# ChenRocks/UNITER

Measured on NVIDIA H100. Metric: uniter_base_encoder_fwd_bwd_samples_per_sec, higher is better.
Workload: dtype bf16

## Files before the change

uniter_b200/csrc/attn.cu:

```cuda
#include "common.h"
#include "ptx.cuh"
#include "wgmma.cuh"

namespace ub {

constexpr int ATT_D = 64;
constexpr int ATT_BM = 128;
constexpr int ATT_BN = 128;
constexpr int ATT_TILE = ATT_BM * ATT_D * 2;
constexpr int ATT_MAXSEQ = 512;
constexpr int ATT_THREADS = 256;

struct AttnParams {
  const int* cu_seqlens;
  int B, H, nheads, T;
  void* ctx;
  float* lse;
  float scale;
  uint32_t drop_thr16;
  float drop_inv_keep;
  uint32_t seed_lo, seed_hi, stream_lo, stream_hi;
  const void* dctx;
  void* dqkv;
  float* dbias;
  const unsigned long long* rng_dev;
};


__device__ __forceinline__ void frag_colsum64_atomic(const float (&d)[32], bool ok0, bool ok1, float* dst,
                                                     int lane) {
#pragma unroll
  for (int jj = 0; jj < 8; ++jj) {
#pragma unroll
    for (int t = 0; t < 2; ++t) {
      float x = (ok0 ? d[4 * jj + t] : 0.f) + (ok1 ? d[4 * jj + 2 + t] : 0.f);
      x += __shfl_xor_sync(0xffffffffu, x, 4);
      x += __shfl_xor_sync(0xffffffffu, x, 8);
      x += __shfl_xor_sync(0xffffffffu, x, 16);
      if (lane < 4) atomicAdd(dst + 8 * jj + 2 * lane + t, x);
    }
  }
}

__device__ __forceinline__ void frag_colsum64_warp(const float (&d)[32], bool ok0, bool ok1, float* dst, int lane) {
#pragma unroll
  for (int jj = 0; jj < 8; ++jj) {
#pragma unroll
    for (int t = 0; t < 2; ++t) {
      float x = (ok0 ? d[4 * jj + t] : 0.f) + (ok1 ? d[4 * jj + 2 + t] : 0.f);
      x += __shfl_xor_sync(0xffffffffu, x, 4);
      x += __shfl_xor_sync(0xffffffffu, x, 8);
      x += __shfl_xor_sync(0xffffffffu, x, 16);
      if (lane < 4) dst[8 * jj + 2 * lane + t] += x;
    }
  }
}

template <bool kBF16>
__device__ __forceinline__ void store_frag_row(void* out_row, const float (&d)[32], int e, int q4, float mul) {
  uint32_t* o = reinterpret_cast<uint32_t*>(out_row);
#pragma unroll
  for (int jj = 0; jj < 8; ++jj)
    o[(8 * jj + 2 * q4) >> 1] = Elem<kBF16>::pack(d[4 * jj + 2 * e] * mul, d[4 * jj + 2 * e + 1] * mul);
}

__device__ __forceinline__ uint64_t attn_drop_group(int bh, int q, int key8) {
  return ((static_cast<uint64_t>(bh) * ATT_MAXSEQ + q) * ATT_MAXSEQ + key8) >> 3;
}

__device__ __forceinline__ void quad_drop_words(const DropoutRng& rng, int bh, int q, int key_base, int jb,
                                                int lane, uint32_t (&w)[4]) {
  const int q4 = lane & 3;
  const uint4 r = rng.draw8(attn_drop_group(bh, q, key_base + 8 * (4 * jb + q4)));
  uint32_t got[4];
#pragma unroll
  for (int k = 0; k < 4; ++k) {
    const int sw = (q4 - k) & 3;
    const uint32_t v = sw == 0 ? r.x : (sw == 1 ? r.y : (sw == 2 ? r.z : r.w));
    got[k] = __shfl_sync(0xffffffffu, v, (lane & ~3) | ((q4 + k) & 3));
  }
#pragma unroll
  for (int t = 0; t < 4; ++t) {
    const int k = (t - q4) & 3;
    w[t] = k == 0 ? got[0] : (k == 1 ? got[1] : (k == 2 ? got[2] : got[3]));
  }
}

__device__ __forceinline__ uint32_t rand16_half(uint32_t w, int t) { return t ? (w >> 16) : (w & 0xFFFFu); }

__device__ __forceinline__ void st_swz128_u32(uint8_t* base, int r, int col, uint32_t v) {
  const int slab = col >> 6;
  const int chunk = (col & 63) >> 3;
  uint8_t* p = base + slab * ATT_TILE + r * 128 + ((chunk ^ (r & 7)) << 4) + (col & 7) * 2;
  *reinterpret_cast<uint32_t*>(p) = v;
}

template <bool kBF16>
__device__ __forceinline__ void row_delta_lse(const AttnParams& p, int seq0, int head, int row, bool ok, int q4,
                                              float& delta, float& lse2) {
  using T16 = typename Elem<kBF16>::T;
  float d = 0.f;
  lse2 = 0.f;
  if (ok) {
    const size_t off = static_cast<size_t>(seq0 + row) * p.H + head * ATT_D + 16 * q4;
    const uint4* g_do = reinterpret_cast<const uint4*>(reinterpret_cast<const T16*>(p.dctx) + off);
    const uint4* g_o = reinterpret_cast<const uint4*>(reinterpret_cast<const T16*>(p.ctx) + off);
#pragma unroll
    for (int v = 0; v < 2; ++v) {
      const uint4 a = __ldg(g_do + v), o = __ldg(g_o + v);
      float2 x, y;
      x = Elem<kBF16>::unpack(a.x); y = Elem<kBF16>::unpack(o.x); d += x.x * y.x + x.y * y.y;
      x = Elem<kBF16>::unpack(a.y); y = Elem<kBF16>::unpack(o.y); d += x.x * y.x + x.y * y.y;
      x = Elem<kBF16>::unpack(a.z); y = Elem<kBF16>::unpack(o.z); d += x.x * y.x + x.y * y.y;
      x = Elem<kBF16>::unpack(a.w); y = Elem<kBF16>::unpack(o.w); d += x.x * y.x + x.y * y.y;
    }
    lse2 = p.lse[static_cast<size_t>(head) * p.T + seq0 + row] * 1.4426950408889634f;
  }
  d += __shfl_xor_sync(0xffffffffu, d, 1);
  d += __shfl_xor_sync(0xffffffffu, d, 2);
  delta = d;
}

constexpr int SH_TILE = 64 * ATT_D * 2;
constexpr int SH_THREADS = 128;
constexpr int SH_MAXSEQ = 128;

__device__ __forceinline__ void wg_sync() { asm volatile("bar.sync 1, 128;" ::: "memory"); }

__device__ __forceinline__ int seq_blocks(const int* cu, int b) { return min((cu[b + 1] - cu[b] + 63) >> 6, 2); }

struct ShortSched {
  const int* cu;
  int B, nheads, h, b;
  long long start, hi;

  __device__ bool valid() const { return h < nheads && start < hi; }
  __device__ int blocks() const { return seq_blocks(cu, b); }

  __device__ void init(const int* cu_, int B_, int nheads_, int lane) {
    cu = cu_; B = B_; nheads = nheads_;
    h = nheads; start = hi = 0;
    int wb = 0;
    for (int b0 = 0; b0 < B; b0 += 32) {
      int c = b0 + lane < B ? seq_blocks(cu, b0 + lane) : 0;
      c *= c;
#pragma unroll
      for (int d = 16; d >= 1; d >>= 1) c += __shfl_xor_sync(0xffffffffu, c, d);
      wb += c;
    }
    if (wb == 0) return;
    const long long W = static_cast<long long>(nheads) * wb;
    const long long lo = W * blockIdx.x / gridDim.x;
    hi = W * (blockIdx.x + 1) / gridDim.x;
    if (lo >= hi) return;
    const int hh = static_cast<int>(lo / wb);
    const long long r = lo - static_cast<long long>(hh) * wb;
    int pref = 0;
    for (int b0 = 0; b0 < B; b0 += 32) {
      int c = b0 + lane < B ? seq_blocks(cu, b0 + lane) : 0;
      c *= c;
      int incl = c;
#pragma unroll
      for (int d = 1; d < 32; d <<= 1) {
        const int t = __shfl_up_sync(0xffffffffu, incl, d);
        if (lane >= d) incl += t;
      }
      const int excl = pref + incl - c;
      const unsigned m = __ballot_sync(0xffffffffu, b0 + lane < B && excl >= r);
      if (m) {
        const int L = __ffs(m) - 1;
        h = hh;
        b = b0 + L;
        start = static_cast<long long>(hh) * wb + __shfl_sync(0xffffffffu, excl, L);
        skip_empty();
        return;
      }
      pref += __shfl_sync(0xffffffffu, incl, 31);
    }
    h = hh + 1;
    b = 0;
    start = static_cast<long long>(h) * wb;
    skip_empty();
  }
  __device__ void step() {
    const int nb = blocks();
    start += nb * nb;
    if (++b == B) { b = 0; ++h; }
  }
  __device__ void skip_empty() {
    while (valid() && cu[b + 1] == cu[b]) step();
  }
  __device__ void next() { step(); skip_empty(); }
};

template <bool kBF16, int NB>
__device__ __forceinline__ void attn_fwd_short_rows(const AttnParams& p, uint32_t uQ, uint32_t uK, uint32_t uV,
                                                    int qb, int S, int seq0, int head, int bh,
                                                    const DropoutRng& rng, int warp, int lane) {
  const int q4 = lane & 3;
  const float c = p.scale * 1.4426950408889634f;
  int qrow[2];
#pragma unroll
  for (int e = 0; e < 2; ++e) qrow[e] = 64 * qb + 16 * warp + (lane >> 2) + 8 * e;

  float s[NB][32];
  wgmma_fence();
#pragma unroll
  for (int kb = 0; kb < NB; ++kb)
#pragma unroll
    for (int k = 0; k < ATT_D / 16; ++k)
      Wgmma<64, kBF16, 0, 0>::ss(s[kb], gmma_desc(uQ + qb * SH_TILE + k * 32, 16, 1024),
                                 gmma_desc(uK + kb * SH_TILE + k * 32, 16, 1024), k != 0);
  wgmma_commit();
  wgmma_wait<0>();

  float m[2] = {-INFINITY, -INFINITY}, l[2] = {0.f, 0.f};
#pragma unroll
  for (int kb = 0; kb < NB; ++kb)
#pragma unroll
    for (int i = 0; i < 32; ++i) {
      const int key = 64 * kb + 8 * (i >> 2) + 2 * q4 + (i & 1);
      if (key < S) m[(i >> 1) & 1] = fmaxf(m[(i >> 1) & 1], s[kb][i]);
    }
#pragma unroll
  for (int e = 0; e < 2; ++e) {
    m[e] = fmaxf(m[e], __shfl_xor_sync(0xffffffffu, m[e], 1));
    m[e] = fmaxf(m[e], __shfl_xor_sync(0xffffffffu, m[e], 2));
  }
  const float mc[2] = {m[0] * c, m[1] * c};

#pragma unroll
  for (int kb = 0; kb < NB; ++kb) {
#pragma unroll
    for (int jb = 0; jb < 2; ++jb) {
      uint32_t dw[2][4];
#pragma unroll
      for (int e = 0; e < 2; ++e)
        if (p.drop_thr16) quad_drop_words(rng, bh, qrow[e], 64 * kb, jb, lane, dw[e]);
#pragma unroll
      for (int jq = 0; jq < 4; ++jq) {
        const int jj = 4 * jb + jq;
#pragma unroll
        for (int e = 0; e < 2; ++e) {
#pragma unroll
          for (int t = 0; t < 2; ++t) {
            const int i = 4 * jj + 2 * e + t;
            const int key = 64 * kb + 8 * jj + 2 * q4 + t;
            float pv = key < S ? ex2_approx(fmaf(s[kb][i], c, -mc[e])) : 0.f;
            l[e] += pv;
            if (p.drop_thr16) {
              const float pr = Elem<kBF16>::to_f(Elem<kBF16>::from_f(pv));
              pv = (rand16_half(dw[e][jq], t) < p.drop_thr16) ? 0.f : pr * p.drop_inv_keep;
            }
            s[kb][i] = pv;
          }
        }
      }
    }
  }

  float o[32];
  wgmma_fence();
#pragma unroll
  for (int kb = 0; kb < NB; ++kb)
#pragma unroll
    for (int kk = 0; kk < 4; ++kk) {
      const uint32_t a[4] = {Elem<kBF16>::pack(s[kb][8 * kk + 0], s[kb][8 * kk + 1]),
                             Elem<kBF16>::pack(s[kb][8 * kk + 2], s[kb][8 * kk + 3]),
                             Elem<kBF16>::pack(s[kb][8 * kk + 4], s[kb][8 * kk + 5]),
                             Elem<kBF16>::pack(s[kb][8 * kk + 6], s[kb][8 * kk + 7])};
      Wgmma<64, kBF16, 0, 1>::rs(o, a, gmma_desc(uV + kb * SH_TILE + kk * 2048, 8192, 1024), (kb | kk) != 0);
    }
  wgmma_commit();
  wgmma_wait<0>();

#pragma unroll
  for (int e = 0; e < 2; ++e) {
    l[e] += __shfl_xor_sync(0xffffffffu, l[e], 1);
    l[e] += __shfl_xor_sync(0xffffffffu, l[e], 2);
    if (qrow[e] >= S) continue;
    if (q4 == 0) p.lse[static_cast<size_t>(head) * p.T + seq0 + qrow[e]] = m[e] * p.scale + logf(l[e]);
    typename Elem<kBF16>::T* out = reinterpret_cast<typename Elem<kBF16>::T*>(p.ctx) +
                                   static_cast<size_t>(seq0 + qrow[e]) * p.H + head * ATT_D;
    store_frag_row<kBF16>(out, o, e, q4, 1.f / l[e]);
  }
}

template <bool kBF16>
__global__ void __launch_bounds__(SH_THREADS, 2)
attn_fwd_short_kernel(const __grid_constant__ CUtensorMap tmQKV64, const AttnParams p) {
  pdl_launch_dependents();
  pdl_wait();
  extern __shared__ __align__(1024) uint8_t smem_raw[];
  uint8_t* smem = smem_raw + ((1024u - (smem_u32(smem_raw) & 1023u)) & 1023u);
  uint8_t* sQ = smem;
  uint8_t* sK = smem + 2 * SH_TILE;
  uint8_t* sV = smem + 4 * SH_TILE;
  uint64_t* bar = reinterpret_cast<uint64_t*>(smem + 6 * SH_TILE);

  const int tid = threadIdx.x, warp = tid >> 5, lane = tid & 31;
  if (tid == 0) {
    tma_prefetch_desc(&tmQKV64);
    mbar_init(&bar[0], 1);
    mbar_init(&bar[1], 1);
    fence_barrier_init();
  }
  wg_sync();
  uint32_t rs0 = p.stream_lo, rs1 = p.stream_hi;
  if (p.drop_thr16) rng_add_dev_offset(p.rng_dev, rs0, rs1);
  DropoutRng rng;
  rng.k0 = p.seed_lo; rng.k1 = p.seed_hi; rng.s0 = rs0; rng.s1 = rs1;

  auto load = [&](const ShortSched& it, int slot) {
    const int seq0 = p.cu_seqlens[it.b], nb = it.blocks(), col = it.h * ATT_D;
    mbar_expect_tx(&bar[slot], nb * 3 * SH_TILE);
    for (int r = 0; r < nb; ++r) {
      const int o = (slot + r) * SH_TILE;
      tma_load_2d(sQ + o, &tmQKV64, &bar[slot], col, seq0 + 64 * r);
      tma_load_2d(sK + o, &tmQKV64, &bar[slot], p.H + col, seq0 + 64 * r);
      tma_load_2d(sV + o, &tmQKV64, &bar[slot], 2 * p.H + col, seq0 + 64 * r);
    }
  };

  ShortSched it;
  it.init(p.cu_seqlens, p.B, p.nheads, lane);
  if (it.valid() && tid == 0) load(it, 0);
  int slot = 0;
  uint32_t ph = 0;
  while (it.valid()) {
    ShortSched nx = it;
    nx.next();
    const int seq0 = p.cu_seqlens[it.b], S = p.cu_seqlens[it.b + 1] - seq0, nb = it.blocks();
    const bool pre = nx.valid() && nb == 1 && nx.blocks() == 1;
    const int nslot = pre ? slot ^ 1 : 0;
    if (pre && tid == 0) load(nx, nslot);
    mbar_wait(&bar[slot], (ph >> slot) & 1);
    ph ^= 1u << slot;
    const uint32_t uQ = smem_u32(sQ + slot * SH_TILE), uK = smem_u32(sK + slot * SH_TILE),
                   uV = smem_u32(sV + slot * SH_TILE);
    const int bh = it.b * p.nheads + it.h;
    if (nb == 1) {
      attn_fwd_short_rows<kBF16, 1>(p, uQ, uK, uV, 0, S, seq0, it.h, bh, rng, warp, lane);
    } else {
#pragma unroll 1
      for (int qb = 0; qb < 2; ++qb)
        attn_fwd_short_rows<kBF16, 2>(p, uQ, uK, uV, qb, S, seq0, it.h, bh, rng, warp, lane);
    }
    wg_sync();
    if (nx.valid() && !pre && tid == 0) load(nx, 0);
    it = nx;
    slot = nslot;
  }
}

constexpr int SH_FWD_SMEM = 6 * SH_TILE + 16 + 1024;

template <bool kBF16, int NB>
__device__ __forceinline__ void dq_block(float (&dq)[32], uint32_t uDS, uint32_t uK, int qb) {
  wgmma_fence();
#pragma unroll
  for (int kk = 0; kk < 4 * NB; ++kk)
    Wgmma<64, kBF16, 0, 1>::ss(dq, gmma_desc(uDS + (qb * NB + (kk >> 2)) * SH_TILE + (kk & 3) * 32, 16, 1024),
                               gmma_desc(uK + kk * 2048, 8192, 1024), kk != 0);
  wgmma_commit();
  wgmma_wait<0>();
}

template <bool kBF16, bool kBias = true>
__global__ void __launch_bounds__(SH_THREADS, 2)
attn_bwd_short_kernel(const __grid_constant__ CUtensorMap tmQKV64, const __grid_constant__ CUtensorMap tmDO64,
                      const AttnParams p) {
  using T16 = typename Elem<kBF16>::T;
  pdl_launch_dependents();
  pdl_wait();
  extern __shared__ __align__(1024) uint8_t smem_raw[];
  __shared__ float sBias[4][3 * ATT_D];
  uint8_t* smem = smem_raw + ((1024u - (smem_u32(smem_raw) & 1023u)) & 1023u);
  uint8_t* sQ = smem;
  uint8_t* sK = smem + 2 * SH_TILE;
  uint8_t* sV = smem + 4 * SH_TILE;
  uint8_t* sdO = smem + 6 * SH_TILE;
  uint8_t* sP = smem + 8 * SH_TILE;
  uint8_t* sDS = smem + 9 * SH_TILE;
  uint64_t* bar = reinterpret_cast<uint64_t*>(smem + 13 * SH_TILE);

  const int tid = threadIdx.x, warp = tid >> 5, lane = tid & 31, q4 = lane & 3;
  if (tid == 0) {
    tma_prefetch_desc(&tmQKV64);
    tma_prefetch_desc(&tmDO64);
    mbar_init(&bar[0], 1);
    mbar_init(&bar[1], 1);
    fence_barrier_init();
  }
  for (int i = tid; i < 4 * 3 * ATT_D; i += SH_THREADS) (&sBias[0][0])[i] = 0.f;
  wg_sync();
  uint32_t rs0 = p.stream_lo, rs1 = p.stream_hi;
  if (p.drop_thr16) rng_add_dev_offset(p.rng_dev, rs0, rs1);
  DropoutRng rng;
  rng.k0 = p.seed_lo; rng.k1 = p.seed_hi; rng.s0 = rs0; rng.s1 = rs1;
  const float c = p.scale * 1.4426950408889634f;
  int r_loc[2];
#pragma unroll
  for (int e = 0; e < 2; ++e) r_loc[e] = 16 * warp + (lane >> 2) + 8 * e;
  const uint32_t uP = smem_u32(sP), uDS = smem_u32(sDS);

  auto load = [&](const ShortSched& it, int slot) {
    const int seq0 = p.cu_seqlens[it.b], nb = it.blocks(), col = it.h * ATT_D;
    mbar_expect_tx(&bar[slot], nb * 4 * SH_TILE);
    for (int r = 0; r < nb; ++r) {
      const int o = (slot + r) * SH_TILE;
      tma_load_2d(sQ + o, &tmQKV64, &bar[slot], col, seq0 + 64 * r);
      tma_load_2d(sK + o, &tmQKV64, &bar[slot], p.H + col, seq0 + 64 * r);
      tma_load_2d(sV + o, &tmQKV64, &bar[slot], 2 * p.H + col, seq0 + 64 * r);
      tma_load_2d(sdO + o, &tmDO64, &bar[slot], col, seq0 + 64 * r);
    }
  };

  ShortSched it;
  it.init(p.cu_seqlens, p.B, p.nheads, lane);
  if (it.valid() && tid == 0) load(it, 0);
  int slot = 0;
  uint32_t ph = 0;
  while (it.valid()) {
    ShortSched nx = it;
    nx.next();
    const int seq0 = p.cu_seqlens[it.b], S = p.cu_seqlens[it.b + 1] - seq0, nb = it.blocks();
    const int head = it.h, bh = it.b * p.nheads + head;
    const bool pre = nx.valid() && nb == 1 && nx.blocks() == 1;
    const int nslot = pre ? slot ^ 1 : 0;
    if (pre && tid == 0) load(nx, nslot);
    mbar_wait(&bar[slot], (ph >> slot) & 1);
    ph ^= 1u << slot;
    const uint32_t uQ = smem_u32(sQ + slot * SH_TILE), udO = smem_u32(sdO + slot * SH_TILE),
                   uK = smem_u32(sK + slot * SH_TILE), uV = smem_u32(sV + slot * SH_TILE);

    for (int kb = 0; kb < nb; ++kb) {
      float dv[32], dk[32];
      for (int qb = 0; qb < nb; ++qb) {
        int qrow[2];
        bool q_ok[2];
        float delta[2], lse2[2];
#pragma unroll
        for (int e = 0; e < 2; ++e) {
          qrow[e] = 64 * qb + r_loc[e];
          q_ok[e] = qrow[e] < S;
          row_delta_lse<kBF16>(p, seq0, head, qrow[e], q_ok[e], q4, delta[e], lse2[e]);
        }
        float s[32], dp[32];
        wgmma_fence();
#pragma unroll
        for (int k = 0; k < ATT_D / 16; ++k)
          Wgmma<64, kBF16, 0, 0>::ss(s, gmma_desc(uQ + qb * SH_TILE + k * 32, 16, 1024),
                                     gmma_desc(uK + kb * SH_TILE + k * 32, 16, 1024), k != 0);
#pragma unroll
        for (int k = 0; k < ATT_D / 16; ++k)
          Wgmma<64, kBF16, 0, 0>::ss(dp, gmma_desc(udO + qb * SH_TILE + k * 32, 16, 1024),
                                     gmma_desc(uV + kb * SH_TILE + k * 32, 16, 1024), k != 0);
        wgmma_commit();
        wgmma_wait<0>();

        uint8_t* dsTile = sDS + (qb * nb + kb) * SH_TILE;
#pragma unroll
        for (int jb = 0; jb < 2; ++jb) {
          uint32_t dw[2][4];
#pragma unroll
          for (int e = 0; e < 2; ++e)
            if (p.drop_thr16) quad_drop_words(rng, bh, qrow[e], 64 * kb, jb, lane, dw[e]);
#pragma unroll
          for (int jq = 0; jq < 4; ++jq) {
            const int jj = 4 * jb + jq;
#pragma unroll
            for (int e = 0; e < 2; ++e) {
              float pd[2], ds[2];
#pragma unroll
              for (int t = 0; t < 2; ++t) {
                const int idx = 4 * jj + 2 * e + t;
                const bool ok = q_ok[e] && 64 * kb + 8 * jj + 2 * q4 + t < S;
                float pr = ok ? ex2_approx(fmaf(s[idx], c, -lse2[e])) : 0.f;
                pr = Elem<kBF16>::to_f(Elem<kBF16>::from_f(pr));
                float dpv = dp[idx];
                float pdv = pr;
                if (p.drop_thr16) {
                  const bool drop = rand16_half(dw[e][jq], t) < p.drop_thr16;
                  pdv = drop ? 0.f : pr * p.drop_inv_keep;
                  dpv = drop ? 0.f : dpv * p.drop_inv_keep;
                }
                pd[t] = pdv;
                ds[t] = ok ? pr * (dpv - delta[e]) * p.scale : 0.f;
              }
              st_swz128_u32(sP, r_loc[e], 8 * jj + 2 * q4, Elem<kBF16>::pack(pd[0], pd[1]));
              st_swz128_u32(dsTile, r_loc[e], 8 * jj + 2 * q4, Elem<kBF16>::pack(ds[0], ds[1]));
            }
          }
        }
        fence_proxy_async_smem();
        wg_sync();

        const uint32_t uDSt = smem_u32(dsTile);
        wgmma_fence();
#pragma unroll
        for (int kk = 0; kk < 4; ++kk)
          Wgmma<64, kBF16, 1, 1>::ss(dv, gmma_desc(uP + kk * 2048, SH_TILE, 1024),
                                     gmma_desc(udO + qb * SH_TILE + kk * 2048, 8192, 1024), (qb | kk) != 0);
#pragma unroll
        for (int kk = 0; kk < 4; ++kk)
          Wgmma<64, kBF16, 1, 1>::ss(dk, gmma_desc(uDSt + kk * 2048, SH_TILE, 1024),
                                     gmma_desc(uQ + qb * SH_TILE + kk * 2048, 8192, 1024), (qb | kk) != 0);
        wgmma_commit();
        wgmma_wait<0>();
        wg_sync();
      }
      int key[2];
      bool k_ok[2];
#pragma unroll
      for (int e = 0; e < 2; ++e) {
        key[e] = 64 * kb + r_loc[e];
        k_ok[e] = key[e] < S;
      }
      if (kBias && p.dbias) {
        frag_colsum64_warp(dk, k_ok[0], k_ok[1], sBias[warp] + ATT_D, lane);
        frag_colsum64_warp(dv, k_ok[0], k_ok[1], sBias[warp] + 2 * ATT_D, lane);
      }
#pragma unroll
      for (int e = 0; e < 2; ++e) {
        if (!k_ok[e]) continue;
        T16* outk = reinterpret_cast<T16*>(p.dqkv) + static_cast<size_t>(seq0 + key[e]) * (3 * p.H) + p.H +
                    head * ATT_D;
        store_frag_row<kBF16>(outk, dk, e, q4, 1.f);
        store_frag_row<kBF16>(outk + p.H, dv, e, q4, 1.f);
      }
    }

    for (int qb = 0; qb < nb; ++qb) {
      float dq[32];
      if (nb == 1) dq_block<kBF16, 1>(dq, uDS, uK, 0);
      else dq_block<kBF16, 2>(dq, uDS, uK, qb);
      bool q_ok[2];
#pragma unroll
      for (int e = 0; e < 2; ++e) q_ok[e] = 64 * qb + r_loc[e] < S;
      if (kBias && p.dbias) frag_colsum64_warp(dq, q_ok[0], q_ok[1], sBias[warp], lane);
#pragma unroll
      for (int e = 0; e < 2; ++e)
        if (q_ok[e])
          store_frag_row<kBF16>(reinterpret_cast<T16*>(p.dqkv) + static_cast<size_t>(seq0 + 64 * qb + r_loc[e]) *
                                                                       (3 * p.H) + head * ATT_D,
                                dq, e, q4, 1.f);
    }
    wg_sync();
    if (nx.valid() && !pre && tid == 0) load(nx, 0);
    if (kBias && p.dbias && (!nx.valid() || nx.h != head)) {
      for (int i = tid; i < 3 * ATT_D; i += SH_THREADS) {
        atomicAdd(p.dbias + (i >> 6) * p.H + head * ATT_D + (i & 63),
                  (sBias[0][i] + sBias[1][i]) + (sBias[2][i] + sBias[3][i]));
        sBias[0][i] = sBias[1][i] = sBias[2][i] = sBias[3][i] = 0.f;
      }
    }
    it = nx;
    slot = nslot;
  }
}

constexpr int SH_BWD_SMEM = 13 * SH_TILE + 16 + 1024;

template <bool kBF16>
__device__ __forceinline__ void qk_block(float (&s)[64], uint32_t sA, uint32_t sB, int wg) {
#pragma unroll
  for (int k = 0; k < ATT_D / 16; ++k)
    Wgmma<128, kBF16, 0, 0>::ss(s, gmma_desc(sA + wg * (64 * 128) + k * 32, 16, 1024),
                                gmma_desc(sB + k * 32, 16, 1024), k != 0);
}

template <bool kBF16>
__global__ void __launch_bounds__(ATT_THREADS, 1)
attn_fwd_kernel(const __grid_constant__ CUtensorMap tmQKV, const AttnParams p) {
  pdl_launch_dependents();
  pdl_wait();
  const int b = blockIdx.z, qt = blockIdx.x;
  const int seq0 = p.cu_seqlens[b];
  const int S = p.cu_seqlens[b + 1] - seq0;
  if (qt * ATT_BM >= S) return;
  const int head = blockIdx.y;
  const int nkv = (S + ATT_BN - 1) / ATT_BN;
  uint32_t rs0 = p.stream_lo, rs1 = p.stream_hi;
  if (p.drop_thr16) rng_add_dev_offset(p.rng_dev, rs0, rs1);

  extern __shared__ __align__(1024) uint8_t smem_raw[];
  uint8_t* smem = smem_raw + ((1024u - (smem_u32(smem_raw) & 1023u)) & 1023u);
  uint8_t* sQ = smem;
  uint8_t* sK = smem + ATT_TILE;
  uint8_t* sV = smem + 2 * ATT_TILE;
  uint64_t* bar_load = reinterpret_cast<uint64_t*>(smem + 3 * ATT_TILE);

  const int tid = threadIdx.x, warp = tid >> 5, lane = tid & 31;
  const int wg = warp >> 2, q4 = lane & 3;
  if (tid == 0) {
    tma_prefetch_desc(&tmQKV);
    mbar_init(bar_load, 1);
    fence_barrier_init();
  }
  __syncthreads();

  int qrow[2];
  bool q_ok[2];
#pragma unroll
  for (int e = 0; e < 2; ++e) {
    qrow[e] = qt * ATT_BM + 64 * wg + 16 * (warp & 3) + (lane >> 2) + 8 * e;
    q_ok[e] = qrow[e] < S;
  }
  const int bh = b * p.nheads + head;
  const float c = p.scale * 1.4426950408889634f;
  const uint32_t uQ = smem_u32(sQ), uK = smem_u32(sK), uV = smem_u32(sV);
  uint32_t ph_load = 0;
  float s[64];

  float m[2] = {-INFINITY, -INFINITY}, l[2] = {0.f, 0.f};
  for (int j = 0; j < nkv; ++j) {
    const int kv_len = min(ATT_BN, S - j * ATT_BN);
    if (tid == 0) {
      const bool with_v = (nkv == 1);
      mbar_expect_tx(bar_load, (j == 0 ? ATT_TILE : 0) + ATT_TILE + (with_v ? ATT_TILE : 0));
      if (j == 0) tma_load_2d(sQ, &tmQKV, bar_load, head * ATT_D, seq0 + qt * ATT_BM);
      tma_load_2d(sK, &tmQKV, bar_load, p.H + head * ATT_D, seq0 + j * ATT_BN);
      if (with_v) tma_load_2d(sV, &tmQKV, bar_load, 2 * p.H + head * ATT_D, seq0 + j * ATT_BN);
    }
    mbar_wait(bar_load, ph_load);
    ph_load ^= 1;
    wgmma_fence();
    qk_block<kBF16>(s, uQ, uK, wg);
    wgmma_commit();
    wgmma_wait<0>();
#pragma unroll
    for (int i = 0; i < 64; ++i) {
      const int key = 8 * (i >> 2) + 2 * q4 + (i & 1);
      if (key < kv_len) m[(i >> 1) & 1] = fmaxf(m[(i >> 1) & 1], s[i]);
    }
    if (nkv > 1) __syncthreads();
  }
#pragma unroll
  for (int e = 0; e < 2; ++e) {
    m[e] = fmaxf(m[e], __shfl_xor_sync(0xffffffffu, m[e], 1));
    m[e] = fmaxf(m[e], __shfl_xor_sync(0xffffffffu, m[e], 2));
  }
  const float mc[2] = {m[0] * c, m[1] * c};

  float o[32];
#pragma unroll
  for (int i = 0; i < 32; ++i) o[i] = 0.f;
  for (int j = 0; j < nkv; ++j) {
    const int kv_len = min(ATT_BN, S - j * ATT_BN);
    if (nkv > 1) {
      if (tid == 0) {
        mbar_expect_tx(bar_load, 2 * ATT_TILE);
        tma_load_2d(sK, &tmQKV, bar_load, p.H + head * ATT_D, seq0 + j * ATT_BN);
        tma_load_2d(sV, &tmQKV, bar_load, 2 * p.H + head * ATT_D, seq0 + j * ATT_BN);
      }
      mbar_wait(bar_load, ph_load);
      ph_load ^= 1;
      wgmma_fence();
      qk_block<kBF16>(s, uQ, uK, wg);
      wgmma_commit();
      wgmma_wait<0>();
    }
    DropoutRng rng;
    rng.k0 = p.seed_lo; rng.k1 = p.seed_hi; rng.s0 = rs0; rng.s1 = rs1;
#pragma unroll
    for (int jb = 0; jb < 4; ++jb) {
      uint32_t dw[2][4];
#pragma unroll
      for (int e = 0; e < 2; ++e)
        if (p.drop_thr16) quad_drop_words(rng, bh, qrow[e], j * ATT_BN, jb, lane, dw[e]);
#pragma unroll
      for (int jq = 0; jq < 4; ++jq) {
        const int jj = 4 * jb + jq;
#pragma unroll
        for (int e = 0; e < 2; ++e) {
#pragma unroll
          for (int t = 0; t < 2; ++t) {
            const int i = 4 * jj + 2 * e + t;
            const int key = 8 * jj + 2 * q4 + t;
            float pv = key < kv_len ? ex2_approx(fmaf(s[i], c, -mc[e])) : 0.f;
            l[e] += pv;
            if (p.drop_thr16) {
              const float pr = Elem<kBF16>::to_f(Elem<kBF16>::from_f(pv));
              pv = (rand16_half(dw[e][jq], t) < p.drop_thr16) ? 0.f : pr * p.drop_inv_keep;
            }
            s[i] = pv;
          }
        }
      }
    }
    wgmma_fence();
#pragma unroll
    for (int kk = 0; kk < ATT_BN / 16; ++kk) {
      const uint32_t a[4] = {Elem<kBF16>::pack(s[8 * kk + 0], s[8 * kk + 1]),
                             Elem<kBF16>::pack(s[8 * kk + 2], s[8 * kk + 3]),
                             Elem<kBF16>::pack(s[8 * kk + 4], s[8 * kk + 5]),
                             Elem<kBF16>::pack(s[8 * kk + 6], s[8 * kk + 7])};
      Wgmma<64, kBF16, 0, 1>::rs(o, a, gmma_desc(uV + kk * 2048, 8192, 1024), (j | kk) != 0);
    }
    wgmma_commit();
    wgmma_wait<0>();
    if (nkv > 1) __syncthreads();
  }

#pragma unroll
  for (int e = 0; e < 2; ++e) {
    l[e] += __shfl_xor_sync(0xffffffffu, l[e], 1);
    l[e] += __shfl_xor_sync(0xffffffffu, l[e], 2);
    if (!q_ok[e]) continue;
    if (q4 == 0) p.lse[static_cast<size_t>(head) * p.T + seq0 + qrow[e]] = m[e] * p.scale + logf(l[e]);
    typename Elem<kBF16>::T* out = reinterpret_cast<typename Elem<kBF16>::T*>(p.ctx) +
                                   static_cast<size_t>(seq0 + qrow[e]) * p.H + head * ATT_D;
    store_frag_row<kBF16>(out, o, e, q4, 1.f / l[e]);
  }
}

constexpr int ATT_FWD_SMEM = 3 * ATT_TILE + 64 + 1024;

template <bool kBF16>
__global__ void __launch_bounds__(ATT_THREADS, 1)
attn_bwd_kernel(const __grid_constant__ CUtensorMap tmQKV, const __grid_constant__ CUtensorMap tmDO,
                const AttnParams p, float* dq_accum) {
  using T16 = typename Elem<kBF16>::T;
  pdl_launch_dependents();
  pdl_wait();
  const int b = blockIdx.z, j = blockIdx.x;
  const int seq0 = p.cu_seqlens[b];
  const int S = p.cu_seqlens[b + 1] - seq0;
  if (j * ATT_BN >= S) return;
  const int head = blockIdx.y;
  const int nq = (S + ATT_BM - 1) / ATT_BM;
  const int nkv = (S + ATT_BN - 1) / ATT_BN;
  uint32_t rs0 = p.stream_lo, rs1 = p.stream_hi;
  if (p.drop_thr16) rng_add_dev_offset(p.rng_dev, rs0, rs1);
  const int kv_len = min(ATT_BN, S - j * ATT_BN);

  extern __shared__ __align__(1024) uint8_t smem_raw[];
  uint8_t* smem = smem_raw + ((1024u - (smem_u32(smem_raw) & 1023u)) & 1023u);
  uint8_t* sQ = smem;
  uint8_t* sdO = smem + ATT_TILE;
  uint8_t* sK = smem + 2 * ATT_TILE;
  uint8_t* sV = smem + 3 * ATT_TILE;
  uint8_t* sP = smem + 4 * ATT_TILE;
  uint8_t* sDS = smem + 6 * ATT_TILE;
  uint64_t* bar_load = reinterpret_cast<uint64_t*>(smem + 8 * ATT_TILE);

  const int tid = threadIdx.x, warp = tid >> 5, lane = tid & 31;
  const int wg = warp >> 2, q4 = lane & 3;
  if (tid == 0) {
    tma_prefetch_desc(&tmQKV);
    tma_prefetch_desc(&tmDO);
    mbar_init(bar_load, 1);
    fence_barrier_init();
  }
  __syncthreads();
  int r_loc[2];
#pragma unroll
  for (int e = 0; e < 2; ++e) r_loc[e] = 64 * wg + 16 * (warp & 3) + (lane >> 2) + 8 * e;
  const int bh = b * p.nheads + head;
  const float c = p.scale * 1.4426950408889634f;
  const uint32_t uQ = smem_u32(sQ), udO = smem_u32(sdO), uK = smem_u32(sK), uV = smem_u32(sV);
  const uint32_t uP = smem_u32(sP), uDS = smem_u32(sDS);
  uint32_t ph_load = 0;
  float dv[32], dk[32];
#pragma unroll
  for (int i = 0; i < 32; ++i) { dv[i] = 0.f; dk[i] = 0.f; }

  for (int i = 0; i < nq; ++i) {
    int qrow[2];
    bool q_ok[2];
#pragma unroll
    for (int e = 0; e < 2; ++e) {
      qrow[e] = i * ATT_BM + r_loc[e];
      q_ok[e] = qrow[e] < S;
    }
    if (tid == 0) {
      mbar_expect_tx(bar_load, (i == 0 ? 4 : 2) * ATT_TILE);
      tma_load_2d(sQ, &tmQKV, bar_load, head * ATT_D, seq0 + i * ATT_BM);
      tma_load_2d(sdO, &tmDO, bar_load, head * ATT_D, seq0 + i * ATT_BM);
      if (i == 0) {
        tma_load_2d(sK, &tmQKV, bar_load, p.H + head * ATT_D, seq0 + j * ATT_BN);
        tma_load_2d(sV, &tmQKV, bar_load, 2 * p.H + head * ATT_D, seq0 + j * ATT_BN);
      }
    }

    float delta[2], lse2[2];
#pragma unroll
    for (int e = 0; e < 2; ++e) row_delta_lse<kBF16>(p, seq0, head, qrow[e], q_ok[e], q4, delta[e], lse2[e]);

    mbar_wait(bar_load, ph_load);
    ph_load ^= 1;
    float s[64], dp[64];
    wgmma_fence();
    qk_block<kBF16>(s, uQ, uK, wg);
    qk_block<kBF16>(dp, udO, uV, wg);
    wgmma_commit();
    wgmma_wait<0>();

    DropoutRng rng;
    rng.k0 = p.seed_lo; rng.k1 = p.seed_hi; rng.s0 = rs0; rng.s1 = rs1;
#pragma unroll
    for (int jb = 0; jb < 4; ++jb) {
      uint32_t dw[2][4];
#pragma unroll
      for (int e = 0; e < 2; ++e)
        if (p.drop_thr16) quad_drop_words(rng, bh, qrow[e], j * ATT_BN, jb, lane, dw[e]);
#pragma unroll
      for (int jq = 0; jq < 4; ++jq) {
        const int jj = 4 * jb + jq;
#pragma unroll
        for (int e = 0; e < 2; ++e) {
          float pd[2], ds[2];
#pragma unroll
          for (int t = 0; t < 2; ++t) {
            const int idx = 4 * jj + 2 * e + t;
            const int key = 8 * jj + 2 * q4 + t;
            const bool ok = q_ok[e] && key < kv_len;
            float pr = ok ? ex2_approx(fmaf(s[idx], c, -lse2[e])) : 0.f;
            pr = Elem<kBF16>::to_f(Elem<kBF16>::from_f(pr));
            float dpv = dp[idx];
            float pdv = pr;
            if (p.drop_thr16) {
              const bool drop = rand16_half(dw[e][jq], t) < p.drop_thr16;
              pdv = drop ? 0.f : pr * p.drop_inv_keep;
              dpv = drop ? 0.f : dpv * p.drop_inv_keep;
            }
            pd[t] = pdv;
            ds[t] = ok ? pr * (dpv - delta[e]) * p.scale : 0.f;
          }
          st_swz128_u32(sP, r_loc[e], 8 * jj + 2 * q4, Elem<kBF16>::pack(pd[0], pd[1]));
          st_swz128_u32(sDS, r_loc[e], 8 * jj + 2 * q4, Elem<kBF16>::pack(ds[0], ds[1]));
        }
      }
    }
    fence_proxy_async_smem();
    __syncthreads();

    float dq[32];
    wgmma_fence();
#pragma unroll
    for (int kk = 0; kk < ATT_BM / 16; ++kk)
      Wgmma<64, kBF16, 1, 1>::ss(dv, gmma_desc(uP + wg * ATT_TILE + kk * 2048, ATT_TILE, 1024),
                                 gmma_desc(udO + kk * 2048, 8192, 1024), (i | kk) != 0);
#pragma unroll
    for (int kk = 0; kk < ATT_BM / 16; ++kk)
      Wgmma<64, kBF16, 1, 1>::ss(dk, gmma_desc(uDS + wg * ATT_TILE + kk * 2048, ATT_TILE, 1024),
                                 gmma_desc(uQ + kk * 2048, 8192, 1024), (i | kk) != 0);
#pragma unroll
    for (int kk = 0; kk < ATT_BN / 16; ++kk)
      Wgmma<64, kBF16, 0, 1>::ss(dq, gmma_desc(uDS + (kk >> 2) * ATT_TILE + wg * (64 * 128) + (kk & 3) * 32, 16, 1024),
                                 gmma_desc(uK + kk * 2048, 8192, 1024), kk != 0);
    wgmma_commit();
    wgmma_wait<0>();
    if (p.dbias)
      frag_colsum64_atomic(dq, q_ok[0], q_ok[1], p.dbias + head * ATT_D, lane);
#pragma unroll
    for (int e = 0; e < 2; ++e) {
      if (!q_ok[e]) continue;
      if (nkv == 1) {
        store_frag_row<kBF16>(reinterpret_cast<T16*>(p.dqkv) + static_cast<size_t>(seq0 + qrow[e]) * (3 * p.H) +
                                  head * ATT_D, dq, e, q4, 1.f);
      } else {
        float* acc = dq_accum + static_cast<size_t>(seq0 + qrow[e]) * p.H + head * ATT_D;
#pragma unroll
        for (int jj = 0; jj < 8; ++jj) {
          atomicAdd(acc + 8 * jj + 2 * q4, dq[4 * jj + 2 * e]);
          atomicAdd(acc + 8 * jj + 2 * q4 + 1, dq[4 * jj + 2 * e + 1]);
        }
      }
    }
    if (i + 1 < nq) __syncthreads();
  }

  int key[2];
  bool k_ok[2];
#pragma unroll
  for (int e = 0; e < 2; ++e) {
    key[e] = j * ATT_BN + r_loc[e];
    k_ok[e] = key[e] < S;
  }
  if (p.dbias) {
    frag_colsum64_atomic(dk, k_ok[0], k_ok[1], p.dbias + p.H + head * ATT_D, lane);
    frag_colsum64_atomic(dv, k_ok[0], k_ok[1], p.dbias + 2 * p.H + head * ATT_D, lane);
  }
#pragma unroll
  for (int e = 0; e < 2; ++e) {
    if (!k_ok[e]) continue;
    T16* outk = reinterpret_cast<T16*>(p.dqkv) + static_cast<size_t>(seq0 + key[e]) * (3 * p.H) + p.H +
                head * ATT_D;
    store_frag_row<kBF16>(outk, dk, e, q4, 1.f);
    store_frag_row<kBF16>(outk + p.H, dv, e, q4, 1.f);
  }
}

template <bool kBF16>
__global__ void attn_dq_convert_kernel(const float* __restrict__ acc, void* dqkv,
                                       const int* __restrict__ cu_seqlens, int H) {
  pdl_launch_dependents();
  pdl_wait();
  const int seq0 = cu_seqlens[blockIdx.x];
  const int S = cu_seqlens[blockIdx.x + 1] - seq0;
  if (S <= ATT_BN) return;
  const int nvec = S * H / 8;
  for (int v = threadIdx.x; v < nvec; v += blockDim.x) {
    const int row = (v * 8) / H, col = (v * 8) % H;
    const float* src = acc + static_cast<size_t>(seq0 + row) * H + col;
    const float4 a = *reinterpret_cast<const float4*>(src);
    const float4 b = *reinterpret_cast<const float4*>(src + 4);
    uint4 u;
    u.x = Elem<kBF16>::pack(a.x, a.y); u.y = Elem<kBF16>::pack(a.z, a.w);
    u.z = Elem<kBF16>::pack(b.x, b.y); u.w = Elem<kBF16>::pack(b.z, b.w);
    *reinterpret_cast<uint4*>(reinterpret_cast<typename Elem<kBF16>::T*>(dqkv) +
                              static_cast<size_t>(seq0 + row) * 3 * H + col) = u;
  }
}

constexpr int ATT_BWD_SMEM = 8 * ATT_TILE + 64 + 1024;

static AttnParams attn_params(const ub200_attn_args& a) {
  AttnParams p{};
  p.cu_seqlens = a.cu_seqlens;
  p.B = a.batch; p.H = a.hidden; p.nheads = a.num_heads; p.T = a.total_tokens;
  p.ctx = a.ctx; p.lse = a.lse;
  p.scale = 0.125f;
  if (a.dropout_p > 0.f) {
    const DropoutThreshold d = dropout_threshold(a.dropout_p);
    p.drop_thr16 = d.thr16;
    p.drop_inv_keep = d.inv_keep;
  } else {
    p.drop_thr16 = 0; p.drop_inv_keep = 1.f;
  }
  p.seed_lo = static_cast<uint32_t>(a.rng_seed); p.seed_hi = static_cast<uint32_t>(a.rng_seed >> 32);
  p.stream_lo = static_cast<uint32_t>(a.rng_stream);
  p.stream_hi = static_cast<uint32_t>(a.rng_stream >> 32);
  p.rng_dev = reinterpret_cast<const unsigned long long*>(a.rng_offset_dev);
  return p;
}

static dim3 short_grid(const ub200_attn_args& a, int per_sm) {
  const long long items = static_cast<long long>(a.batch) * a.num_heads;
  const long long g = static_cast<long long>(num_sms()) * per_sm;
  return dim3(static_cast<unsigned>(g < items ? g : items));
}

}

extern "C" int ub200_attn_fwd(const ub200_attn_args* args, ub200_stream_t stream_) {
  using namespace ub;
  UB_CHECK_ARG(args != nullptr, "attn_fwd: args is NULL");
  const ub200_attn_args& a = *args;
  cudaStream_t stream = reinterpret_cast<cudaStream_t>(stream_);
  UB_CHECK_ARG(a.qkv && a.ctx && a.lse && a.cu_seqlens, "attn_fwd: null pointer");
  UB_CHECK_ARG(a.batch > 0 && a.total_tokens > 0, "attn_fwd: empty batch");
  UB_CHECK_ARG(a.num_heads > 0 && a.hidden == a.num_heads * ATT_D,
               "attn_fwd: head_dim must be 64 (hidden=%d heads=%d)", a.hidden, a.num_heads);
  UB_CHECK_ARG(a.max_seqlen > 0 && a.max_seqlen <= ATT_MAXSEQ,
               "attn_fwd: max_seqlen %d outside (0, %d]", a.max_seqlen, ATT_MAXSEQ);
  UB_CHECK_ARG(a.dtype == UB200_F16 || a.dtype == UB200_BF16, "attn_fwd: bad dtype");
  UB_CHECK_ARG(a.dropout_p >= 0.f && a.dropout_p < 1.f, "attn_fwd: dropout_p out of range");

  const AttnParams p = attn_params(a);
  const bool bf = a.dtype == UB200_BF16;
  CUtensorMap tm;
  if (a.max_seqlen <= SH_MAXSEQ) {
    int rc = make_tma_2d(&tm, a.qkv, a.dtype, a.total_tokens, 3 * a.hidden, 3 * a.hidden, 64, ATT_D);
    if (rc) return rc;
    void (*kern)(const CUtensorMap, const AttnParams) = bf ? attn_fwd_short_kernel<true> : attn_fwd_short_kernel<false>;
    static unsigned long long configured[2] = {0, 0};
    if (first_use_on_device(configured[bf ? 1 : 0]))
      UB_CHECK_CUDA(cudaFuncSetAttribute(kern, cudaFuncAttributeMaxDynamicSharedMemorySize, SH_FWD_SMEM));
    ProfScope ps(stream);
    UB_CHECK_CUDA(launch_pdl(kern, short_grid(a, 2), dim3(SH_THREADS), SH_FWD_SMEM, stream, 1, tm, p));
  } else {
    int rc = make_tma_2d(&tm, a.qkv, a.dtype, a.total_tokens, 3 * a.hidden, 3 * a.hidden, ATT_BM, ATT_D);
    if (rc) return rc;
    dim3 grid((a.max_seqlen + ATT_BM - 1) / ATT_BM, a.num_heads, a.batch);
    void (*kern)(const CUtensorMap, const AttnParams) = bf ? attn_fwd_kernel<true> : attn_fwd_kernel<false>;
    static unsigned long long configured[2] = {0, 0};
    if (first_use_on_device(configured[bf ? 1 : 0]))
      UB_CHECK_CUDA(cudaFuncSetAttribute(kern, cudaFuncAttributeMaxDynamicSharedMemorySize, ATT_FWD_SMEM));
    ProfScope ps(stream);
    UB_CHECK_CUDA(launch_pdl(kern, grid, dim3(ATT_THREADS), ATT_FWD_SMEM, stream, 1, tm, p));
  }
  UB_CHECK_CUDA(cudaGetLastError());
  return 0;
}

extern "C" int64_t ub200_attn_bwd_workspace_bytes(int32_t total_tokens, int32_t hidden,
                                                  int32_t max_seqlen) {
  if (max_seqlen <= ub::ATT_BN) return 0;
  return static_cast<int64_t>(total_tokens) * hidden * 4;
}

extern "C" int ub200_attn_bwd(const ub200_attn_args* args, ub200_stream_t stream_) {
  using namespace ub;
  UB_CHECK_ARG(args != nullptr, "attn_bwd: args is NULL");
  const ub200_attn_args& a = *args;
  cudaStream_t stream = reinterpret_cast<cudaStream_t>(stream_);
  UB_CHECK_ARG(a.qkv && a.ctx && a.lse && a.cu_seqlens && a.dctx && a.dqkv, "attn_bwd: null pointer");
  UB_CHECK_ARG(a.batch > 0 && a.total_tokens > 0, "attn_bwd: empty batch");
  UB_CHECK_ARG(a.num_heads > 0 && a.hidden == a.num_heads * ATT_D, "attn_bwd: head_dim must be 64");
  UB_CHECK_ARG(a.max_seqlen > 0 && a.max_seqlen <= ATT_MAXSEQ, "attn_bwd: max_seqlen %d outside (0, %d]",
               a.max_seqlen, ATT_MAXSEQ);
  UB_CHECK_ARG(a.dtype == UB200_F16 || a.dtype == UB200_BF16, "attn_bwd: bad dtype");
  const bool multi = a.max_seqlen > ATT_BN;
  UB_CHECK_ARG(!multi || a.workspace, "attn_bwd: max_seqlen > 128 needs the dQ workspace");

  AttnParams p = attn_params(a);
  p.dctx = a.dctx; p.dqkv = a.dqkv; p.dbias = a.dbias;
  const int di = a.dtype == UB200_BF16 ? 1 : 0;

  if (deterministic()) {
    if (a.max_seqlen > SH_MAXSEQ)
      return set_error(UB200_EUNSUPPORTED, "attn_bwd: deterministic mode supports max_seqlen <= %d (got %d)",
                       SH_MAXSEQ, a.max_seqlen);
    CUtensorMap tmQ, tmD;
    int rc = make_tma_2d(&tmQ, a.qkv, a.dtype, a.total_tokens, 3 * a.hidden, 3 * a.hidden, 64, ATT_D);
    if (rc) return rc;
    rc = make_tma_2d(&tmD, a.dctx, a.dtype, a.total_tokens, a.hidden, a.hidden, 64, ATT_D);
    if (rc) return rc;
    p.dbias = nullptr;
    void (*kern)(const CUtensorMap, const CUtensorMap, const AttnParams) =
        di ? attn_bwd_short_kernel<true, false> : attn_bwd_short_kernel<false, false>;
    static unsigned long long configured[2] = {0, 0};
    if (first_use_on_device(configured[di]))
      UB_CHECK_CUDA(cudaFuncSetAttribute(kern, cudaFuncAttributeMaxDynamicSharedMemorySize, SH_BWD_SMEM));
    {
      ProfScope ps(stream);
      UB_CHECK_CUDA(launch_pdl(kern, short_grid(a, 2), dim3(SH_THREADS), SH_BWD_SMEM, stream, 1, tmQ, tmD, p));
    }
    UB_CHECK_CUDA(cudaGetLastError());
    if (a.dbias)
      return launch_colsum_det(a.dtype, a.dqkv, a.dbias, a.total_tokens, 3 * a.hidden, 3 * a.hidden, stream,
                               a.cu_seqlens + a.batch);
    return 0;
  }

  if (a.max_seqlen <= SH_MAXSEQ) {
    CUtensorMap tmQ, tmD;
    int rc = make_tma_2d(&tmQ, a.qkv, a.dtype, a.total_tokens, 3 * a.hidden, 3 * a.hidden, 64, ATT_D);
    if (rc) return rc;
    rc = make_tma_2d(&tmD, a.dctx, a.dtype, a.total_tokens, a.hidden, a.hidden, 64, ATT_D);
    if (rc) return rc;
    void (*kern)(const CUtensorMap, const CUtensorMap, const AttnParams) =
        di ? attn_bwd_short_kernel<true> : attn_bwd_short_kernel<false>;
    static unsigned long long configured[2] = {0, 0};
    if (first_use_on_device(configured[di]))
      UB_CHECK_CUDA(cudaFuncSetAttribute(kern, cudaFuncAttributeMaxDynamicSharedMemorySize, SH_BWD_SMEM));
    ProfScope ps(stream);
    UB_CHECK_CUDA(launch_pdl(kern, short_grid(a, 2), dim3(SH_THREADS), SH_BWD_SMEM, stream, 1, tmQ, tmD, p));
    UB_CHECK_CUDA(cudaGetLastError());
    return 0;
  }

  CUtensorMap tmQ, tmD;
  int rc = make_tma_2d(&tmQ, a.qkv, a.dtype, a.total_tokens, 3 * a.hidden, 3 * a.hidden, ATT_BM, ATT_D);
  if (rc) return rc;
  rc = make_tma_2d(&tmD, a.dctx, a.dtype, a.total_tokens, a.hidden, a.hidden, ATT_BM, ATT_D);
  if (rc) return rc;
  float* acc = reinterpret_cast<float*>(a.workspace);
  UB_CHECK_CUDA(cudaMemsetAsync(acc, 0, static_cast<size_t>(a.total_tokens) * a.hidden * 4, stream));

  dim3 grid((a.max_seqlen + ATT_BN - 1) / ATT_BN, a.num_heads, a.batch);
  void (*kern)(const CUtensorMap, const CUtensorMap, const AttnParams, float*) =
      di ? attn_bwd_kernel<true> : attn_bwd_kernel<false>;
  static unsigned long long configured[2] = {0, 0};
  if (first_use_on_device(configured[di]))
    UB_CHECK_CUDA(cudaFuncSetAttribute(kern, cudaFuncAttributeMaxDynamicSharedMemorySize, ATT_BWD_SMEM));
  {
    ProfScope ps(stream);
    UB_CHECK_CUDA(launch_pdl(kern, grid, dim3(ATT_THREADS), ATT_BWD_SMEM, stream, 1, tmQ, tmD, p, acc));
  }
  UB_CHECK_CUDA(cudaGetLastError());
  {
    ProfScope ps(stream);
    if (di) UB_CHECK_CUDA(launch_pdl(attn_dq_convert_kernel<true>, dim3(a.batch), dim3(256), 0, stream, 1, static_cast<const float*>(acc), a.dqkv, a.cu_seqlens, a.hidden));
    else UB_CHECK_CUDA(launch_pdl(attn_dq_convert_kernel<false>, dim3(a.batch), dim3(256), 0, stream, 1, static_cast<const float*>(acc), a.dqkv, a.cu_seqlens, a.hidden));
    UB_CHECK_CUDA(cudaGetLastError());
  }
  return 0;
}
```

Measured before the change: 11390.

## Split two-block short-attention fwd into per-query-block work units with cost-weighted scheduling

Sequences of up to 64 rows and those of 65-128 rows get separate weighted costs in the short-attention scheduler. The forward kernel now processes each 64-row query block of a two-block sequence as its own work unit. The forward smem layout becomes two stages, each holding one Q tile plus two K and two V tiles, so the next unit is always prefetched and double buffered. The aim is better load balance across CTAs and full overlap of TMA loads with compute. In the backward kernel, per-row delta/LSE values are computed once per query block and reused across key blocks instead of being reloaded each time. The trade-offs are more smem per stage, K/V reloaded for each query unit, and hand-tuned cost constants.

```diff
diff --git a/uniter_b200/csrc/attn.cu b/uniter_b200/csrc/attn.cu
--- a/uniter_b200/csrc/attn.cu
+++ b/uniter_b200/csrc/attn.cu
@@ -129,21 +129,27 @@
 
 __device__ __forceinline__ int seq_blocks(const int* cu, int b) { return min((cu[b + 1] - cu[b] + 63) >> 6, 2); }
 
+constexpr int SH_FWD_COST1 = 10, SH_FWD_COST2 = 19;
+constexpr int SH_BWD_COST1 = 1, SH_BWD_COST2 = 2;
+
+template <int kCost1, int kCost2, bool kSplit>
 struct ShortSched {
   const int* cu;
-  int B, nheads, h, b;
+  int B, nheads, h, b, qb;
   long long start, hi;
+
+  __device__ static int unit_cost(int nb) { return nb == 0 ? 0 : (nb == 1 ? kCost1 : kCost2); }
+  __device__ static int seq_cost(int nb) { return (kSplit && nb == 2 ? 2 : 1) * unit_cost(nb); }
 
   __device__ bool valid() const { return h < nheads && start < hi; }
   __device__ int blocks() const { return seq_blocks(cu, b); }
 
   __device__ void init(const int* cu_, int B_, int nheads_, int lane) {
     cu = cu_; B = B_; nheads = nheads_;
-    h = nheads; start = hi = 0;
+    h = nheads; qb = 0; start = hi = 0;
     int wb = 0;
     for (int b0 = 0; b0 < B; b0 += 32) {
-      int c = b0 + lane < B ? seq_blocks(cu, b0 + lane) : 0;
-      c *= c;
+      int c = b0 + lane < B ? seq_cost(seq_blocks(cu, b0 + lane)) : 0;
 #pragma unroll
       for (int d = 16; d >= 1; d >>= 1) c += __shfl_xor_sync(0xffffffffu, c, d);
       wb += c;
@@ -157,8 +163,8 @@
     const long long r = lo - static_cast<long long>(hh) * wb;
     int pref = 0;
     for (int b0 = 0; b0 < B; b0 += 32) {
-      int c = b0 + lane < B ? seq_blocks(cu, b0 + lane) : 0;
-      c *= c;
+      const int nb = b0 + lane < B ? seq_blocks(cu, b0 + lane) : 0;
+      const int c = seq_cost(nb), w = unit_cost(nb);
       int incl = c;
 #pragma unroll
       for (int d = 1; d < 32; d <<= 1) {
@@ -166,12 +172,14 @@
         if (lane >= d) incl += t;
       }
       const int excl = pref + incl - c;
-      const unsigned m = __ballot_sync(0xffffffffu, b0 + lane < B && excl >= r);
+      const unsigned m = __ballot_sync(0xffffffffu, b0 + lane < B && excl + c - w >= r);
       if (m) {
         const int L = __ffs(m) - 1;
+        const int ex = __shfl_sync(0xffffffffu, excl, L), wl = __shfl_sync(0xffffffffu, w, L);
         h = hh;
         b = b0 + L;
-        start = static_cast<long long>(hh) * wb + __shfl_sync(0xffffffffu, excl, L);
+        qb = ex >= r ? 0 : 1;
+        start = static_cast<long long>(hh) * wb + ex + qb * wl;
         skip_empty();
         return;
       }
@@ -184,7 +192,12 @@
   }
   __device__ void step() {
     const int nb = blocks();
-    start += nb * nb;
+    start += unit_cost(nb);
+    if (kSplit && nb == 2 && qb == 0) {
+      qb = 1;
+      return;
+    }
+    qb = 0;
     if (++b == B) { b = 0; ++h; }
   }
   __device__ void skip_empty() {
@@ -192,6 +205,9 @@
   }
   __device__ void next() { step(); skip_empty(); }
 };
+
+using FwdSched = ShortSched<SH_FWD_COST1, SH_FWD_COST2, true>;
+using BwdSched = ShortSched<SH_BWD_COST1, SH_BWD_COST2, false>;
 
 template <bool kBF16, int NB>
 __device__ __forceinline__ void attn_fwd_short_rows(const AttnParams& p, uint32_t uQ, uint32_t uK, uint32_t uV,
@@ -286,6 +302,8 @@
   }
 }
 
+constexpr int SH_FWD_STAGE = 5 * SH_TILE;
+
 template <bool kBF16>
 __global__ void __launch_bounds__(SH_THREADS, 2)
 attn_fwd_short_kernel(const __grid_constant__ CUtensorMap tmQKV64, const AttnParams p) {
@@ -293,10 +311,7 @@
   pdl_wait();
   extern __shared__ __align__(1024) uint8_t smem_raw[];
   uint8_t* smem = smem_raw + ((1024u - (smem_u32(smem_raw) & 1023u)) & 1023u);
-  uint8_t* sQ = smem;
-  uint8_t* sK = smem + 2 * SH_TILE;
-  uint8_t* sV = smem + 4 * SH_TILE;
-  uint64_t* bar = reinterpret_cast<uint64_t*>(smem + 6 * SH_TILE);
+  uint64_t* bar = reinterpret_cast<uint64_t*>(smem + 2 * SH_FWD_STAGE);
 
   const int tid = threadIdx.x, warp = tid >> 5, lane = tid & 31;
   if (tid == 0) {
@@ -311,49 +326,41 @@
   DropoutRng rng;
   rng.k0 = p.seed_lo; rng.k1 = p.seed_hi; rng.s0 = rs0; rng.s1 = rs1;
 
-  auto load = [&](const ShortSched& it, int slot) {
-    const int seq0 = p.cu_seqlens[it.b], nb = it.blocks(), col = it.h * ATT_D;
-    mbar_expect_tx(&bar[slot], nb * 3 * SH_TILE);
+  auto load = [&](const FwdSched& u, int st) {
+    const int seq0 = p.cu_seqlens[u.b], nb = u.blocks(), col = u.h * ATT_D;
+    uint8_t* s = smem + st * SH_FWD_STAGE;
+    mbar_expect_tx(&bar[st], (1 + 2 * nb) * SH_TILE);
+    tma_load_2d(s, &tmQKV64, &bar[st], col, seq0 + 64 * u.qb);
     for (int r = 0; r < nb; ++r) {
-      const int o = (slot + r) * SH_TILE;
-      tma_load_2d(sQ + o, &tmQKV64, &bar[slot], col, seq0 + 64 * r);
-      tma_load_2d(sK + o, &tmQKV64, &bar[slot], p.H + col, seq0 + 64 * r);
-      tma_load_2d(sV + o, &tmQKV64, &bar[slot], 2 * p.H + col, seq0 + 64 * r);
+      tma_load_2d(s + (1 + r) * SH_TILE, &tmQKV64, &bar[st], p.H + col, seq0 + 64 * r);
+      tma_load_2d(s + (3 + r) * SH_TILE, &tmQKV64, &bar[st], 2 * p.H + col, seq0 + 64 * r);
     }
   };
 
-  ShortSched it;
+  FwdSched it;
   it.init(p.cu_seqlens, p.B, p.nheads, lane);
   if (it.valid() && tid == 0) load(it, 0);
-  int slot = 0;
+  int st = 0;
   uint32_t ph = 0;
   while (it.valid()) {
-    ShortSched nx = it;
+    FwdSched nx = it;
     nx.next();
-    const int seq0 = p.cu_seqlens[it.b], S = p.cu_seqlens[it.b + 1] - seq0, nb = it.blocks();
-    const bool pre = nx.valid() && nb == 1 && nx.blocks() == 1;
-    const int nslot = pre ? slot ^ 1 : 0;
-    if (pre && tid == 0) load(nx, nslot);
-    mbar_wait(&bar[slot], (ph >> slot) & 1);
-    ph ^= 1u << slot;
-    const uint32_t uQ = smem_u32(sQ + slot * SH_TILE), uK = smem_u32(sK + slot * SH_TILE),
-                   uV = smem_u32(sV + slot * SH_TILE);
+    if (nx.valid() && tid == 0) load(nx, st ^ 1);
+    const int seq0 = p.cu_seqlens[it.b], S = p.cu_seqlens[it.b + 1] - seq0;
+    mbar_wait(&bar[st], (ph >> st) & 1);
+    ph ^= 1u << st;
+    const uint32_t u = smem_u32(smem + st * SH_FWD_STAGE);
+    const uint32_t uQ = u - it.qb * SH_TILE, uK = u + SH_TILE, uV = u + 3 * SH_TILE;
     const int bh = it.b * p.nheads + it.h;
-    if (nb == 1) {
-      attn_fwd_short_rows<kBF16, 1>(p, uQ, uK, uV, 0, S, seq0, it.h, bh, rng, warp, lane);
-    } else {
-#pragma unroll 1
-      for (int qb = 0; qb < 2; ++qb)
-        attn_fwd_short_rows<kBF16, 2>(p, uQ, uK, uV, qb, S, seq0, it.h, bh, rng, warp, lane);
-    }
+    if (it.blocks() == 1) attn_fwd_short_rows<kBF16, 1>(p, uQ, uK, uV, 0, S, seq0, it.h, bh, rng, warp, lane);
+    else attn_fwd_short_rows<kBF16, 2>(p, uQ, uK, uV, it.qb, S, seq0, it.h, bh, rng, warp, lane);
     wg_sync();
-    if (nx.valid() && !pre && tid == 0) load(nx, 0);
     it = nx;
-    slot = nslot;
-  }
-}
-
-constexpr int SH_FWD_SMEM = 6 * SH_TILE + 16 + 1024;
+    st ^= 1;
+  }
+}
+
+constexpr int SH_FWD_SMEM = 2 * SH_FWD_STAGE + 16 + 1024;
 
 template <bool kBF16, int NB>
 __device__ __forceinline__ void dq_block(float (&dq)[32], uint32_t uDS, uint32_t uK, int qb) {
@@ -404,7 +411,7 @@
   for (int e = 0; e < 2; ++e) r_loc[e] = 16 * warp + (lane >> 2) + 8 * e;
   const uint32_t uP = smem_u32(sP), uDS = smem_u32(sDS);
 
-  auto load = [&](const ShortSched& it, int slot) {
+  auto load = [&](const BwdSched& it, int slot) {
     const int seq0 = p.cu_seqlens[it.b], nb = it.blocks(), col = it.h * ATT_D;
     mbar_expect_tx(&bar[slot], nb * 4 * SH_TILE);
     for (int r = 0; r < nb; ++r) {
@@ -416,13 +423,13 @@
     }
   };
 
-  ShortSched it;
+  BwdSched it;
   it.init(p.cu_seqlens, p.B, p.nheads, lane);
   if (it.valid() && tid == 0) load(it, 0);
   int slot = 0;
   uint32_t ph = 0;
   while (it.valid()) {
-    ShortSched nx = it;
+    BwdSched nx = it;
     nx.next();
     const int seq0 = p.cu_seqlens[it.b], S = p.cu_seqlens[it.b + 1] - seq0, nb = it.blocks();
     const int head = it.h, bh = it.b * p.nheads + head;
@@ -434,6 +441,7 @@
     const uint32_t uQ = smem_u32(sQ + slot * SH_TILE), udO = smem_u32(sdO + slot * SH_TILE),
                    uK = smem_u32(sK + slot * SH_TILE), uV = smem_u32(sV + slot * SH_TILE);
 
+    float delta0[2] = {}, lse20[2] = {}, delta1[2] = {}, lse21[2] = {};
     for (int kb = 0; kb < nb; ++kb) {
       float dv[32], dk[32];
       for (int qb = 0; qb < nb; ++qb) {
@@ -444,7 +452,18 @@
         for (int e = 0; e < 2; ++e) {
           qrow[e] = 64 * qb + r_loc[e];
           q_ok[e] = qrow[e] < S;
-          row_delta_lse<kBF16>(p, seq0, head, qrow[e], q_ok[e], q4, delta[e], lse2[e]);
+        }
+        if (kb == 0) {
+#pragma unroll
+          for (int e = 0; e < 2; ++e) {
+            if (qb == 0) row_delta_lse<kBF16>(p, seq0, head, qrow[e], q_ok[e], q4, delta0[e], lse20[e]);
+            else row_delta_lse<kBF16>(p, seq0, head, qrow[e], q_ok[e], q4, delta1[e], lse21[e]);
+          }
+        }
+#pragma unroll
+        for (int e = 0; e < 2; ++e) {
+          delta[e] = qb ? delta1[e] : delta0[e];
+          lse2[e] = qb ? lse21[e] : lse20[e];
         }
         float s[32], dp[32];
         wgmma_fence();
```

After: 11650, median of 6. +2.3%, better.
